# silencht/SG-SLAM

Hardware: AMD Instinct MI355X
Metric: tracked frames/sec (640x480 RGB-D) (higher is better)
Workload: dtype u8/f32(bf16x3 matrix products)/f64

## Files before the change

### sg_slam_amd/csrc/sgx_flow_kernels.h

```cpp
#pragma once
#include "sgx_rt.h"
#include "sgx_block.h"
#include "sgx_lane.h"
#include <float.h>
#include <math.h>

#define SGX_LK_MAXL 4
#define SGX_LK_WIN 21
#define SGX_LK_TILE_PITCH 36
struct SgxLkGeom {
    int nl;
    int w[SGX_LK_MAXL], h[SGX_LK_MAXL], pitch[SGX_LK_MAXL];
    unsigned ioff[SGX_LK_MAXL];
    unsigned img_stride;
};

SGX_DEV int sgx_reflect101(int p, int len)
{
    if (len == 1) return 0;
    while (p < 0 || p >= len) { if (p < 0) p = -p; else p = 2 * len - 2 - p; }
    return p;
}
SGX_DEV int sgx_floor_f(float v) { return (int)floorf(v); }
SGX_DEV float sgx_i64_to_f32(long long v)
// ... 118 lines not shown
    k.w10 = sgx_cvround((1.f - a) * b * (float)(1 << 14));
    k.w11 = (1 << 14) - k.w00 - k.w01 - k.w10;
    return k;
}
#define SGX_LK_DESCALE(x, n) (((x) + (1 << ((n) - 1))) >> (n))

struct SgxLkStep { float dx, dy; };
SGX_DEV SgxLkStep sgx_lk_step(float A11, float A12, float A22, float D, long long sb1, long long sb2)
{
    const float FLT_SCALE = 1.f / (1 << 20);
    const float b1 = sgx_i64_to_f32(sb1) * FLT_SCALE, b2 = sgx_i64_to_f32(sb2) * FLT_SCALE;
    SgxLkStep s;
    s.dx = (A12 * b2 - A22 * b1) * D;
    s.dy = (A12 * b1 - A11 * b2) * D;
    return s;
}

struct SgxLkArgs {
    const uint8_t *cur_img, *prev_img;
    const uint8_t *keys; const int *n; int cap;
    float *prev_xy; uint8_t *status;
    int max_count; double eps2; float min_eig;
    int batch, kblocks;
};
SGX_DEV void sgx_lk_decode_block(int i, int batch, int kblocks, int &f, int &kb)
{
    const int full = (batch / 8) * 8;
    if (i < full * kblocks) { const int x = i & 7, j = i >> 3; kb = j % kblocks; f = x + 8 * (j / kblocks); }
    else { const int j = i - full * kblocks; f = full + j / kblocks; kb = j % kblocks; }
}

#ifdef SGX_EMU
static inline int sgx_lk_px(const uint8_t *I, int w, int h, int pitch, int x, int y) { return I[(size_t)sgx_reflect101(y, h) * pitch + sgx_reflect101(x, w)]; }
static void sgx_lk_track_point(const SgxLkGeom &g, const uint8_t *I0, const uint8_t *J0, float kx, float ky, int max_count, double eps2, float min_eig,
                               float *ox, float *oy, uint8_t *ost)
{
    const int W = SGX_LK_WIN; const float half = (W - 1) * 0.5f, FLT_SCALE = 1.f / (1 << 20);
    float outx = 0.f, outy = 0.f; uint8_t status = 1;
    static thread_local short Iw[SGX_LK_WIN * SGX_LK_WIN], dIw[SGX_LK_WIN * SGX_LK_WIN * 2];
    for (int level = g.nl - 1; level >= 0; level--) {
        const int w = g.w[level], h = g.h[level], pitch = g.pitch[level];
        const uint8_t *I = I0 + g.ioff[level], *J = J0 + g.ioff[level];
        const float sc = 1.0f / (float)(1 << level);
        float prevx = kx * sc, prevy = ky * sc, nextx, nexty;
        if (level == g.nl - 1) { nextx = prevx; nexty = prevy; } else { nextx = outx * 2.f; nexty = outy * 2.f; }
        outx = nextx; outy = nexty;
        prevx -= half; prevy -= half;
        const int ipx = sgx_floor_f(prevx), ipy = sgx_floor_f(prevy);
        if (ipx < -W || ipx >= w || ipy < -W || ipy >= h) { if (level == 0) status = 0; continue; }
        SgxLkWeights k = sgx_lk_weights(prevx - ipx, prevy - ipy);
        long long s11 = 0, s12 = 0, s22 = 0;
        for (int y = 0; y < W; y++) for (int x = 0; x < W; x++) {
            int pv[4], dx[4], dy[4];
            for (int c = 0; c < 4; c++) {
                const int gx = ipx + x + (c & 1), gy = ipy + y + (c >> 1);
                pv[c] = sgx_lk_px(I, w, h, pitch, gx, gy);
                if (gx < 0 || gy < 0 || gx >= w || gy >= h) { dx[c] = dy[c] = 0; }
                else {
                    int t0[3], t1[3];
                    for (int q = 0; q < 3; q++) {
                        const int a = sgx_lk_px(I, w, h, pitch, gx - 1 + q, gy - 1), b = sgx_lk_px(I, w, h, pitch, gx - 1 + q, gy), cc = sgx_lk_px(I, w, h, pitch, gx - 1 + q, gy + 1);
                        t0[q] = (a + cc) * 3 + b * 10; t1[q] = cc - a;
                    }
                    dx[c] = t0[2] - t0[0]; dy[c] = (t1[0] + t1[2]) * 3 + t1[1] * 10;
                }
            }
            const int iv = SGX_LK_DESCALE(pv[0] * k.w00 + pv[1] * k.w01 + pv[2] * k.w10 + pv[3] * k.w11, 9);
            const int ix = SGX_LK_DESCALE(dx[0] * k.w00 + dx[1] * k.w01 + dx[2] * k.w10 + dx[3] * k.w11, 14);
            const int iy = SGX_LK_DESCALE(dy[0] * k.w00 + dy[1] * k.w01 + dy[2] * k.w10 + dy[3] * k.w11, 14);
            Iw[y * W + x] = (short)iv; dIw[(y * W + x) * 2] = (short)ix; dIw[(y * W + x) * 2 + 1] = (short)iy;
            s11 += (long long)ix * ix; s12 += (long long)ix * iy; s22 += (long long)iy * iy;
        }
        const float A11 = sgx_i64_to_f32(s11) * FLT_SCALE, A12 = sgx_i64_to_f32(s12) * FLT_SCALE, A22 = sgx_i64_to_f32(s22) * FLT_SCALE;
        float D = A11 * A22 - A12 * A12;
        const float minEig = (A22 + A11 - sqrtf((A11 - A22) * (A11 - A22) + 4.f * A12 * A12)) / (float)(2 * W * W);
        if (minEig < min_eig || D < FLT_EPSILON) { if (level == 0) status = 0; continue; }
        D = 1.f / D;
        nextx -= half; nexty -= half;
        float pdx = 0.f, pdy = 0.f;
        for (int j = 0; j < max_count; j++) {
            const int inx = sgx_floor_f(nextx), iny = sgx_floor_f(nexty);
            if (inx < -W || inx >= w || iny < -W || iny >= h) { if (level == 0) status = 0; break; }
            k = sgx_lk_weights(nextx - inx, nexty - iny);
            long long sb1 = 0, sb2 = 0;
            for (int y = 0; y < W; y++) for (int x = 0; x < W; x++) {
                int pv[4];
                for (int c = 0; c < 4; c++) pv[c] = sgx_lk_px(J, w, h, pitch, inx + x + (c & 1), iny + y + (c >> 1));
                const int diff = SGX_LK_DESCALE(pv[0] * k.w00 + pv[1] * k.w01 + pv[2] * k.w10 + pv[3] * k.w11, 9) - Iw[y * W + x];
                sb1 += (long long)diff * dIw[(y * W + x) * 2]; sb2 += (long long)diff * dIw[(y * W + x) * 2 + 1];
            }
            const SgxLkStep st = sgx_lk_step(A11, A12, A22, D, sb1, sb2);
            nextx += st.dx; nexty += st.dy;
            outx = nextx + half; outy = nexty + half;
            if ((double)st.dx * st.dx + (double)st.dy * st.dy <= eps2) break;
            if (j > 0 && fabs((double)(st.dx + pdx)) < 0.01 && fabs((double)(st.dy + pdy)) < 0.01) { outx -= st.dx * 0.5f; outy -= st.dy * 0.5f; break; }
            pdx = st.dx; pdy = st.dy;
        }
        if (status && level == 0) {
            const int ix = sgx_floor_f(outx - half), iy = sgx_floor_f(outy - half);
            if (ix < -W || ix >= w || iy < -W || iy >= h) status = 0;
        }
    }
    *ox = outx; *oy = outy; *ost = status;
}
SGX_KERNEL(256) k_lk_track(SgxLkGeom g, SgxLkArgs A)
{
    SGX_THREADS_BEGIN(tid)
    int f, kb;
    sgx_lk_decode_block((int)blockIdx.x, A.batch, A.kblocks, f, kb);
    const int kp = kb * 4 + (tid >> 6);
    if ((tid & 63) == 0 && kp < A.n[f] && kp < A.cap) {
        const float *kpt = (const float *)(A.keys + ((size_t)f * A.cap + kp) * 28);
        float ox, oy; uint8_t st;
        sgx_lk_track_point(g, A.cur_img + (size_t)f * g.img_stride, A.prev_img + (size_t)f * g.img_stride, kpt[0], kpt[1], A.max_count, A.eps2, A.min_eig, &ox, &oy, &st);
        A.prev_xy[2 * ((size_t)f * A.cap + kp)] = ox; A.prev_xy[2 * ((size_t)f * A.cap + kp) + 1] = oy;
        if (A.status) A.status[(size_t)f * A.cap + kp] = st;
    }
    SGX_THREADS_END
}
#else
SGX_DEV int sgx_wave_sum_i32(int v)
{
    v += __builtin_amdgcn_update_dpp(0, v, 0xB1, 0xF, 0xF, true);
    v += __builtin_amdgcn_update_dpp(0, v, 0x4E, 0xF, 0xF, true);
    v += __builtin_amdgcn_update_dpp(0, v, 0x124, 0xF, 0xF, true);
    v += __builtin_amdgcn_update_dpp(0, v, 0x128, 0xF, 0xF, true);
    v += __builtin_amdgcn_update_dpp(0, v, 0x142, 0xA, 0xF, false);
    v += __builtin_amdgcn_update_dpp(0, v, 0x143, 0xC, 0xF, false);
    return __builtin_amdgcn_readlane(v, 63);
}
SGX_DEV float sgx_wave_sum_f32(int v)
{
    const int lo = sgx_wave_sum_i32(v & 0xFFFF), hi = sgx_wave_sum_i32(v >> 16);
    return fmaf((float)hi, 65536.0f, (float)lo);
}
SGX_DEV int sgx_mul24(int a, int b) { return __mul24(a, b); }
SGX_DEV int sgx_reflect1(int p, int len) { p = p < 0 ? -p : p; p = p >= len ? 2 * len - 2 - p : p; return min(max(p, 0), len - 1); }

typedef short sgx_i16x2 __attribute__((ext_vector_type(2)));
typedef unsigned short sgx_u16x2 __attribute__((ext_vector_type(2)));
SGX_DEV sgx_i16x2 sgx_as_i16x2(uint32_t v) { return __builtin_bit_cast(sgx_i16x2, v); }
SGX_DEV uint32_t sgx_as_u32(sgx_i16x2 v) { return __builtin_bit_cast(uint32_t, v); }
#define SGX_LK_PAIR(hi, lo, a, b) sgx_as_i16x2(__builtin_amdgcn_perm((hi), (lo), (uint32_t)(a) | 0x0c00u | ((uint32_t)(b) << 16) | 0x0c000000u))
SGX_DEV sgx_i16x2 sgx_lk_next(sgx_i16x2 p, sgx_i16x2 q) { return sgx_as_i16x2(__builtin_amdgcn_alignbit(sgx_as_u32(q), sgx_as_u32(p), 16)); }
#if defined(SGX_LK_NODOT) && !defined(SGX_EMU)
SGX_DEV int sgx_lk_dot2_mad(sgx_i16x2 a, sgx_i16x2 b, int c)
{
    const uint32_t ua = __builtin_bit_cast(uint32_t, a), ub = __builtin_bit_cast(uint32_t, b);
    asm("v_mad_i32_i16 %0, %1, %2, %0 op_sel:[0,0,0,0]" : "+v"(c) : "v"(ua), "v"(ub));
    asm("v_mad_i32_i16 %0, %1, %2, %0 op_sel:[1,1,0,0]" : "+v"(c) : "v"(ua), "v"(ub));
    return c;
}
#define SGX_LK_DOT2(a, b, c) sgx_lk_dot2_mad((a), (b), (c))
#else
#define SGX_LK_DOT2(a, b, c) __builtin_amdgcn_sdot2((a), (b), (c), false)
#endif
SGX_DEV int sgx_lk_dot2_keep(sgx_i16x2 a, sgx_i16x2 b, int c) { return SGX_LK_DOT2(a, b, c); }

template <int PASSES>
SGX_DEV void sgx_lk_stage(uint32_t *tile, const uint8_t *img, int w, int h, int pitch, int ox, int oy, int rl, int cl)
{
    __builtin_amdgcn_fence(__ATOMIC_SEQ_CST, "wavefront"); __builtin_amdgcn_wave_barrier();
    const int gx = ox + 4 * cl;
    const bool inside = gx >= 0 && gx + 4 <= w;
    if (rl < 7) {
        uint32_t v[PASSES];
        if (inside) {
#pragma unroll
            for (int p = 0; p < PASSES; p++) v[p] = *(const uint32_t *)(img + (size_t)sgx_reflect1(oy + p * 7 + rl, h) * pitch + gx);
        } else {
            const int x0 = sgx_reflect1(gx, w), x1 = sgx_reflect1(gx + 1, w), x2 = sgx_reflect1(gx + 2, w), x3 = sgx_reflect1(gx + 3, w);
#pragma unroll
            for (int p = 0; p < PASSES; p++) {
                const uint8_t *src = img + (size_t)sgx_reflect1(oy + p * 7 + rl, h) * pitch;
                v[p] = (uint32_t)src[x0] | ((uint32_t)src[x1] << 8) | ((uint32_t)src[x2] << 16) | ((uint32_t)src[x3] << 24);
            }
        }
#pragma unroll
        for (int p = 0; p < PASSES; p++) tile[(p * 7 + rl) * (SGX_LK_TILE_PITCH / 4) + cl] = v[p];
    }
    __builtin_amdgcn_fence(__ATOMIC_SEQ_CST, "wavefront"); __builtin_amdgcn_wave_barrier();
}

#ifdef SGX_DEBUG_TAPS
SGX_KERNEL(256) k_lk_track(SgxLkGeom g, SgxLkArgs A)
{
    __shared__ uint32_t tiles[4][35 * SGX_LK_TILE_PITCH / 4 + 5];
    const int tid = (int)threadIdx.x, lane = tid & 63, wv = tid >> 6;
    int f, kb;
    sgx_lk_decode_block((int)blockIdx.x, A.batch, A.kblocks, f, kb);
    const int kp = kb * 4 + wv;
    if (kp >= A.n[f] || kp >= A.cap) return;
    uint32_t *tile = tiles[wv];
    const uint8_t *tile8 = (const uint8_t *)tile;
    const int W = SGX_LK_WIN; const float half = 10.0f, FLT_SCALE = 1.f / (1 << 20);
    const float *kpt = (const float *)(A.keys + ((size_t)f * A.cap + kp) * 28);
    const float kx = __builtin_bit_cast(float, __builtin_amdgcn_readfirstlane(__builtin_bit_cast(int, kpt[0])));
    const float ky = __builtin_bit_cast(float, __builtin_amdgcn_readfirstlane(__builtin_bit_cast(int, kpt[1])));
    const uint8_t *I0 = A.cur_img + (size_t)f * g.img_stride, *J0 = A.prev_img + (size_t)f * g.img_stride;
    const int r = lane / 3, s7 = (lane - 3 * r) * 7;
    const int rl = lane / 9, cl = lane - 9 * rl;
    const bool active = lane < 63;
    const int lane_off = active ? r * SGX_LK_TILE_PITCH + s7 : 0;
    float outx = 0.f, outy = 0.f; int status = 1;

    for (int level = g.nl - 1; level >= 0; level--) {
        const int w = g.w[level], h = g.h[level], pitch = g.pitch[level];
        const uint8_t *I = I0 + g.ioff[level], *J = J0 + g.ioff[level];
        const float sc = 1.0f / (float)(1 << level);
        float prevx = kx * sc, prevy = ky * sc, nextx, nexty;
        if (level == g.nl - 1) { nextx = prevx; nexty = prevy; } else { nextx = outx * 2.f; nexty = outy * 2.f; }
        outx = nextx; outy = nexty;
        prevx -= half; prevy -= half;
        const int ipx = sgx_floor_f(prevx), ipy = sgx_floor_f(prevy);
        if (ipx < -W || ipx >= w || ipy < -W || ipy >= h) { if (level == 0) status = 0; continue; }
        SgxLkWeights k = sgx_lk_weights(prevx - ipx, prevy - ipy);
        sgx_i16x2 W0 = sgx_as_i16x2((uint32_t)k.w00 | ((uint32_t)k.w01 << 16)), W1 = sgx_as_i16x2((uint32_t)k.w10 | ((uint32_t)k.w11 << 16));

        int ivb[7]; int ix[7], iy[7];
        int s11 = 0, s12 = 0, s22 = 0;
        {
            const int gy0 = ipy + r, gx0 = ipx + s7;
            sgx_i16x2 P[4][5];
            const bool direct = ipx >= 1 && ipx + 25 < w && ipy >= 1 && ipy + 22 < h;
            if (direct) {
                const uint8_t *gb = I + (size_t)(active ? gy0 - 1 : ipy) * pitch + (active ? gx0 - 1 : ipx);
#pragma unroll
                for (int j = 0; j < 4; j++) {
                    uint32_t q[3];
                    __builtin_memcpy(q, gb + (size_t)j * pitch, 12);
                    P[j][0] = SGX_LK_PAIR(q[0], q[0], 0, 1); P[j][1] = SGX_LK_PAIR(q[0], q[0], 2, 3);
                    P[j][2] = SGX_LK_PAIR(q[1], q[1], 0, 1); P[j][3] = SGX_LK_PAIR(q[1], q[1], 2, 3);
                    P[j][4] = SGX_LK_PAIR(q[2], q[2], 0, 1);
                }
            } else {
                const int tx = ((ipx - 1) >> 2) << 2, ty = ipy - 1;
                sgx_lk_stage<4>(tile, I, w, h, pitch, tx, ty, rl, cl);
                const uint8_t *tb = tile8 + lane_off + (ipx - 1 - tx);
#pragma unroll
                for (int j = 0; j < 4; j++) {
                    uint32_t q[3];
                    __builtin_memcpy(q, tb + j * SGX_LK_TILE_PITCH, 12);
                    P[j][0] = SGX_LK_PAIR(q[0], q[0], 0, 1); P[j][1] = SGX_LK_PAIR(q[0], q[0], 2, 3);
                    P[j][2] = SGX_LK_PAIR(q[1], q[1], 0, 1); P[j][3] = SGX_LK_PAIR(q[1], q[1], 2, 3);
                    P[j][4] = SGX_LK_PAIR(q[2], q[2], 0, 1);
                }
            }
            const sgx_i16x2 c3 = { 3, 3 }, c10 = { 10, 10 };
            const sgx_i16x2 Wd0 = active ? W0 : sgx_as_i16x2(0u), Wd1 = active ? W1 : sgx_as_i16x2(0u);
            sgx_i16x2 S0[5], S1[5], D0[5], D1[5];
#pragma unroll
            for (int q = 0; q < 5; q++) {
                S0[q] = (P[0][q] + P[2][q]) * c3 + P[1][q] * c10; D0[q] = P[2][q] - P[0][q];
                S1[q] = (P[1][q] + P[3][q]) * c3 + P[2][q] * c10; D1[q] = P[3][q] - P[1][q];
            }
            sgx_i16x2 xa[5], ya[5], xb[5], yb[5];
            const bool whole = ipx >= 0 && ipx + W < w && ipy >= 0 && ipy + W < h;
#pragma unroll
            for (int q = 0; q < 4; q++) {
                xa[q] = S0[q + 1] - S0[q]; ya[q] = (D0[q] + D0[q + 1]) * c3 + sgx_lk_next(D0[q], D0[q + 1]) * c10;
                xb[q] = S1[q + 1] - S1[q]; yb[q] = (D1[q] + D1[q + 1]) * c3 + sgx_lk_next(D1[q], D1[q + 1]) * c10;
            }
            if (!whole) {
                const bool rowa = gy0 >= 0 && gy0 < h, rowb = gy0 + 1 >= 0 && gy0 + 1 < h;
#pragma unroll
                for (int q = 0; q < 4; q++) {
                    const int x = gx0 + 2 * q;
                    const uint32_t m = ((x >= 0 && x < w) ? 0xFFFFu : 0u) | ((x + 1 >= 0 && x + 1 < w) ? 0xFFFF0000u : 0u);
                    const uint32_t ma = rowa ? m : 0u, mb = rowb ? m : 0u;
                    xa[q] = sgx_as_i16x2(sgx_as_u32(xa[q]) & ma); ya[q] = sgx_as_i16x2(sgx_as_u32(ya[q]) & ma);
                    xb[q] = sgx_as_i16x2(sgx_as_u32(xb[q]) & mb); yb[q] = sgx_as_i16x2(sgx_as_u32(yb[q]) & mb);
                }
            }
#pragma unroll
            for (int c = 0; c < 7; c++) {
                const sgx_i16x2 pxa = (c & 1) ? sgx_lk_next(xa[c >> 1], xa[(c >> 1) + 1]) : xa[c >> 1], pxb = (c & 1) ? sgx_lk_next(xb[c >> 1], xb[(c >> 1) + 1]) : xb[c >> 1];
                const sgx_i16x2 pya = (c & 1) ? sgx_lk_next(ya[c >> 1], ya[(c >> 1) + 1]) : ya[c >> 1], pyb = (c & 1) ? sgx_lk_next(yb[c >> 1], yb[(c >> 1) + 1]) : yb[c >> 1];
                const sgx_i16x2 pia = (c & 1) ? P[1][(c + 1) >> 1] : sgx_lk_next(P[1][c >> 1], P[1][(c >> 1) + 1]), pib = (c & 1) ? P[2][(c + 1) >> 1] : sgx_lk_next(P[2][c >> 1], P[2][(c >> 1) + 1]);
                const int v = SGX_LK_DOT2(pib, W1, SGX_LK_DOT2(pia, W0, 256)) >> 9;
                const int vx = SGX_LK_DOT2(pxb, Wd1, SGX_LK_DOT2(pxa, Wd0, 8192)) >> 14;
                const int vy = SGX_LK_DOT2(pyb, Wd1, SGX_LK_DOT2(pya, Wd0, 8192)) >> 14;
                ivb[c] = 256 - (v << 9); ix[c] = vx; iy[c] = vy;
                s11 += sgx_mul24(vx, vx); s12 += sgx_mul24(vx, vy); s22 += sgx_mul24(vy, vy);
            }
        }
        const float A11 = sgx_wave_sum_f32(s11) * FLT_SCALE, A12 = sgx_wave_sum_f32(s12) * FLT_SCALE, A22 = sgx_wave_sum_f32(s22) * FLT_SCALE;
        float D = A11 * A22 - A12 * A12;
        const float minEig = (A22 + A11 - sqrtf((A11 - A22) * (A11 - A22) + 4.f * A12 * A12)) / (float)(2 * W * W);
        if (minEig < A.min_eig || D < FLT_EPSILON) { if (level == 0) status = 0; continue; }
        D = 1.f / D;
        nextx -= half; nexty -= half;
        float pdx = 0.f, pdy = 0.f;
        int ox = 0, oy = 0; bool staged = false;
        for (int j = 0; j < A.max_count; j++) {
            const int inx = sgx_floor_f(nextx), iny = sgx_floor_f(nexty);
            if (inx < -W || inx >= w || iny < -W || iny >= h) { if (level == 0) status = 0; break; }
            k = sgx_lk_weights(nextx - inx, nexty - iny);
            W0 = sgx_as_i16x2((uint32_t)k.w00 | ((uint32_t)k.w01 << 16)); W1 = sgx_as_i16x2((uint32_t)k.w10 | ((uint32_t)k.w11 << 16));
            if (!staged || inx < ox || inx - ox > SGX_LK_TILE_PITCH - 22 || iny < oy || iny - oy > 35 - 22) {
                ox = ((inx - 5) >> 2) << 2; oy = iny - 6;
                sgx_lk_stage<5>(tile, J, w, h, pitch, ox, oy, rl, cl);
                staged = true;
            }
            int sb1 = 0, sb2 = 0;
            {
                const uint8_t *tb = tile8 + lane_off + (iny - oy) * SGX_LK_TILE_PITCH + (inx - ox);
                uint32_t a[2], b[2];
                __builtin_memcpy(a, tb, 8); __builtin_memcpy(b, tb + SGX_LK_TILE_PITCH, 8);
#pragma unroll
                for (int c = 0; c < 7; c++) {
                    const int diff = SGX_LK_DOT2(SGX_LK_PAIR(b[1], b[0], c, c + 1), W1, SGX_LK_DOT2(SGX_LK_PAIR(a[1], a[0], c, c + 1), W0, ivb[c])) >> 9;
                    sb1 += sgx_mul24(diff, ix[c]); sb2 += sgx_mul24(diff, iy[c]);
                }
            }
            const float b1 = sgx_wave_sum_f32(sb1) * FLT_SCALE, b2 = sgx_wave_sum_f32(sb2) * FLT_SCALE;
            const float dx = (A12 * b2 - A22 * b1) * D, dy = (A12 * b1 - A11 * b2) * D;
            nextx += dx; nexty += dy;
            outx = nextx + half; outy = nexty + half;
            if ((double)dx * dx + (double)dy * dy <= A.eps2) break;
            if (j > 0 && fabs((double)(dx + pdx)) < 0.01 && fabs((double)(dy + pdy)) < 0.01) { outx -= dx * 0.5f; outy -= dy * 0.5f; break; }
            pdx = dx; pdy = dy;
        }
        if (status && level == 0) {
            const int qx = sgx_floor_f(outx - half), qy = sgx_floor_f(outy - half);
            if (qx < -W || qx >= w || qy < -W || qy >= h) status = 0;
        }
    }
    if (lane == 0) {
        A.prev_xy[2 * ((size_t)f * A.cap + kp)] = outx; A.prev_xy[2 * ((size_t)f * A.cap + kp) + 1] = outy;
        if (A.status) A.status[(size_t)f * A.cap + kp] = (uint8_t)status;
    }
}
#endif
#endif

#ifndef SGX_EMU
SGX_DEV int sgx_row_sum_i32(int v)
{
    v += __builtin_amdgcn_update_dpp(v, v, 0xB1, 0xF, 0xF, true);
    v += __builtin_amdgcn_update_dpp(v, v, 0x4E, 0xF, 0xF, true);
    v += __builtin_amdgcn_update_dpp(v, v, 0x124, 0xF, 0xF, true);
    v += __builtin_amdgcn_update_dpp(v, v, 0x128, 0xF, 0xF, true);
    return v;
}
template <int LPK>
SGX_DEV float sgx_group_sum_f32(int v)
{
    int lo = sgx_row_sum_i32(v & 0xFFFF), hi = sgx_row_sum_i32(v >> 16);
    if (LPK == 32) { lo += __shfl_xor(lo, 16, 64); hi += __shfl_xor(hi, 16, 64); }
    return fmaf((float)hi, 65536.0f, (float)lo);
}

#define SGX_LK4_PITCH 32
template <int NROWS, int LPK>
SGX_DEV void sgx_lk_stage_row(uint32_t *tile, const uint8_t *img, int w, int h, int pitch, int ox, int oy, int l16)
{
    constexpr int RPP = LPK / 8, G = LPK == 16 ? 6 : 3;
    const int c = l16 & 7, rs = l16 >> 3, gx = ox + 4 * c;
    const bool inside = gx >= 0 && gx + 4 <= w;
    const int x0 = sgx_reflect1(gx, w), x1 = sgx_reflect1(gx + 1, w), x2 = sgx_reflect1(gx + 2, w), x3 = sgx_reflect1(gx + 3, w);
#pragma unroll 1
    for (int r0 = rs; r0 < NROWS; r0 += RPP * G) {
        uint32_t v[G];
#pragma unroll
        for (int p = 0; p < G; p++) {
            const uint8_t *src = img + (size_t)sgx_reflect1(oy + min(r0 + RPP * p, NROWS - 1), h) * pitch;
            if (inside) v[p] = *(const uint32_t *)(src + gx);
            else v[p] = (uint32_t)src[x0] | ((uint32_t)src[x1] << 8) | ((uint32_t)src[x2] << 16) | ((uint32_t)src[x3] << 24);
        }
#pragma unroll
        for (int p = 0; p < G; p++) { const int r = r0 + RPP * p; if (r < NROWS) tile[r * (SGX_LK4_PITCH / 4) + c] = v[p]; }
    }
}

SGX_DEV void sgx_lk_segment_setup(const sgx_i16x2 (&P)[4][5], sgx_i16x2 W0, sgx_i16x2 W1, bool whole, int gx0, int gy0, int w, int h,
                                  int (&ivb)[7], uint32_t (&ixy)[7], int &s11, int &s12, int &s22)
{
    const sgx_i16x2 c3 = { 3, 3 }, c10 = { 10, 10 };
    sgx_i16x2 S0[5], S1[5], D0[5], D1[5];
#pragma unroll
    for (int q = 0; q < 5; q++) {
        S0[q] = (P[0][q] + P[2][q]) * c3 + P[1][q] * c10; D0[q] = P[2][q] - P[0][q];
        S1[q] = (P[1][q] + P[3][q]) * c3 + P[2][q] * c10; D1[q] = P[3][q] - P[1][q];
    }
    sgx_i16x2 xa[5], ya[5], xb[5], yb[5];
#pragma unroll
    for (int q = 0; q < 4; q++) {
        xa[q] = S0[q + 1] - S0[q]; ya[q] = (D0[q] + D0[q + 1]) * c3 + sgx_lk_next(D0[q], D0[q + 1]) * c10;
        xb[q] = S1[q + 1] - S1[q]; yb[q] = (D1[q] + D1[q + 1]) * c3 + sgx_lk_next(D1[q], D1[q + 1]) * c10;
    }
    if (!whole) {
        const bool rowa = gy0 >= 0 && gy0 < h, rowb = gy0 + 1 >= 0 && gy0 + 1 < h;
#pragma unroll
        for (int q = 0; q < 4; q++) {
            const int x = gx0 + 2 * q;
            const uint32_t m = ((x >= 0 && x < w) ? 0xFFFFu : 0u) | ((x + 1 >= 0 && x + 1 < w) ? 0xFFFF0000u : 0u);
            const uint32_t ma = rowa ? m : 0u, mb = rowb ? m : 0u;
            xa[q] = sgx_as_i16x2(sgx_as_u32(xa[q]) & ma); ya[q] = sgx_as_i16x2(sgx_as_u32(ya[q]) & ma);
            xb[q] = sgx_as_i16x2(sgx_as_u32(xb[q]) & mb); yb[q] = sgx_as_i16x2(sgx_as_u32(yb[q]) & mb);
        }
    }
#pragma unroll
    for (int c = 0; c < 7; c++) {
        const sgx_i16x2 pxa = (c & 1) ? sgx_lk_next(xa[c >> 1], xa[(c >> 1) + 1]) : xa[c >> 1], pxb = (c & 1) ? sgx_lk_next(xb[c >> 1], xb[(c >> 1) + 1]) : xb[c >> 1];
        const sgx_i16x2 pya = (c & 1) ? sgx_lk_next(ya[c >> 1], ya[(c >> 1) + 1]) : ya[c >> 1], pyb = (c & 1) ? sgx_lk_next(yb[c >> 1], yb[(c >> 1) + 1]) : yb[c >> 1];
        const sgx_i16x2 pia = (c & 1) ? P[1][(c + 1) >> 1] : sgx_lk_next(P[1][c >> 1], P[1][(c >> 1) + 1]), pib = (c & 1) ? P[2][(c + 1) >> 1] : sgx_lk_next(P[2][c >> 1], P[2][(c >> 1) + 1]);
        const int v = SGX_LK_DOT2(pib, W1, SGX_LK_DOT2(pia, W0, 256)) >> 9;
        const int vx = SGX_LK_DOT2(pxb, W1, SGX_LK_DOT2(pxa, W0, 8192)) >> 14;
        const int vy = SGX_LK_DOT2(pyb, W1, SGX_LK_DOT2(pya, W0, 8192)) >> 14;
        ivb[c] = 256 - (v << 9); ixy[c] = ((uint32_t)vx & 0xFFFFu) | ((uint32_t)vy << 16);
        s11 += sgx_mul24(vx, vx); s12 += sgx_mul24(vx, vy); s22 += sgx_mul24(vy, vy);
    }
}
SGX_DEV int sgx_mad_lo16(int diff, uint32_t pair, int acc) { asm("v_mad_i32_i16 %0, %1, %2, %0 op_sel:[0,0,0,0]" : "+v"(acc) : "v"(diff), "v"(pair)); return acc; }
SGX_DEV int sgx_mad_hi16(int diff, uint32_t pair, int acc) { asm("v_mad_i32_i16 %0, %1, %2, %0 op_sel:[0,1,0,0]" : "+v"(acc) : "v"(diff), "v"(pair)); return acc; }

template <int KPW>
SGX_KERNEL_OCC(256, (KPW == 4 ? 3 : 5)) k_lk_trackN(SgxLkGeom g, SgxLkArgs A)
{
    constexpr int LPK = 64 / KPW, SPL = KPW;
    constexpr int TD = 36 * SGX_LK4_PITCH / 4 + 5;
    __shared__ uint32_t tiles[4 * KPW][TD];
    const int tid = (int)threadIdx.x, lane = tid & 63, wv = tid >> 6, row = lane / LPK, l16 = lane % LPK;
    int f, kb;
    sgx_lk_decode_block((int)blockIdx.x, A.batch, A.kblocks, f, kb);
    const int nkp = min(A.n[f], A.cap);
    if (kb * (4 * KPW) + wv * KPW >= nkp) return;
    const int kp = kb * (4 * KPW) + wv * KPW + row;
    const bool valid = kp < nkp;
    uint32_t *tile = tiles[wv * KPW + row];
    const uint8_t *tile8 = (const uint8_t *)tile;
    const int W = SGX_LK_WIN; const float half = 10.0f, FLT_SCALE = 1.f / (1 << 20);
    const float *kpt = (const float *)(A.keys + ((size_t)f * A.cap + (valid ? kp : 0)) * 28);
    const float kx = kpt[0], ky = kpt[1];
    const uint8_t *I0 = A.cur_img + (size_t)f * g.img_stride, *J0 = A.prev_img + (size_t)f * g.img_stride;
    int soff[SPL], srow[SPL], scol[SPL];
#pragma unroll
    for (int q = 0; q < SPL; q++) { const int si = min(l16 + LPK * q, 62); srow[q] = si / 3; scol[q] = (si - 3 * srow[q]) * 7; soff[q] = srow[q] * SGX_LK4_PITCH + scol[q]; }
    const bool idle3 = l16 == LPK - 1;
    float outx = 0.f, outy = 0.f; int status = 1;

    for (int level = g.nl - 1; level >= 0; level--) {
        const int w = g.w[level], h = g.h[level], pitch = g.pitch[level];
        const uint8_t *I = I0 + g.ioff[level], *J = J0 + g.ioff[level];
        const float sc = 1.0f / (float)(1 << level);
        float prevx = kx * sc, prevy = ky * sc, nextx, nexty;
        if (level == g.nl - 1) { nextx = prevx; nexty = prevy; } else { nextx = outx * 2.f; nexty = outy * 2.f; }
        outx = nextx; outy = nexty;
        prevx -= half; prevy -= half;
        const int ipx = sgx_floor_f(prevx), ipy = sgx_floor_f(prevy);
        bool act = valid;
        if (ipx < -W || ipx >= w || ipy < -W || ipy >= h) { if (level == 0) status = 0; act = false; }
        if (!__any(act)) continue;
        SgxLkWeights k = sgx_lk_weights(prevx - ipx, prevy - ipy);
        sgx_i16x2 W0 = sgx_as_i16x2((uint32_t)k.w00 | ((uint32_t)k.w01 << 16)), W1 = sgx_as_i16x2((uint32_t)k.w10 | ((uint32_t)k.w11 << 16));

        int ivb[SPL][7]; uint32_t ixy[SPL][7];
        int s11 = 0, s12 = 0, s22 = 0;
        {
            const bool direct = act && ipx >= 1 && ipx + 25 < w && ipy >= 1 && ipy + 22 < h;
            const bool whole = !__any(act && !(ipx >= 0 && ipx + W < w && ipy >= 0 && ipy + W < h));
            const int tx = ((ipx - 1) >> 2) << 2, ty = ipy - 1;
            if (__any(act && !direct)) {
                __builtin_amdgcn_fence(__ATOMIC_SEQ_CST, "wavefront"); __builtin_amdgcn_wave_barrier();
                if (act && !direct) sgx_lk_stage_row<28, LPK>(tile, I, w, h, pitch, tx, ty, l16);
                __builtin_amdgcn_fence(__ATOMIC_SEQ_CST, "wavefront"); __builtin_amdgcn_wave_barrier();
            }
#pragma unroll
            for (int q = 0; q < SPL; q++) {
                const int gy0 = ipy + srow[q], gx0 = ipx + scol[q];
                sgx_i16x2 P[4][5];
                if (direct) {
                    const uint8_t *gb = I + (size_t)(gy0 - 1) * pitch + (gx0 - 1);
#pragma unroll
                    for (int j = 0; j < 4; j++) {
                        uint32_t d[3];
                        __builtin_memcpy(d, gb + (size_t)j * pitch, 12);
                        P[j][0] = SGX_LK_PAIR(d[0], d[0], 0, 1); P[j][1] = SGX_LK_PAIR(d[0], d[0], 2, 3);
                        P[j][2] = SGX_LK_PAIR(d[1], d[1], 0, 1); P[j][3] = SGX_LK_PAIR(d[1], d[1], 2, 3);
                        P[j][4] = SGX_LK_PAIR(d[2], d[2], 0, 1);
                    }
                } else {
                    const uint8_t *tb = tile8 + soff[q] + (ipx - 1 - tx);
#pragma unroll
                    for (int j = 0; j < 4; j++) {
                        uint32_t d[3];
                        __builtin_memcpy(d, tb + j * SGX_LK4_PITCH, 12);
                        P[j][0] = SGX_LK_PAIR(d[0], d[0], 0, 1); P[j][1] = SGX_LK_PAIR(d[0], d[0], 2, 3);
                        P[j][2] = SGX_LK_PAIR(d[1], d[1], 0, 1); P[j][3] = SGX_LK_PAIR(d[1], d[1], 2, 3);
                        P[j][4] = SGX_LK_PAIR(d[2], d[2], 0, 1);
                    }
                }
                const bool on = act && !(q == SPL - 1 && idle3);
                const sgx_i16x2 Wq0 = on ? W0 : sgx_as_i16x2(0u), Wq1 = on ? W1 : sgx_as_i16x2(0u);
                sgx_lk_segment_setup(P, Wq0, Wq1, whole, gx0, gy0, w, h, ivb[q], ixy[q], s11, s12, s22);
                __builtin_amdgcn_sched_barrier(0);
            }
        }
        const float A11 = sgx_group_sum_f32<LPK>(s11) * FLT_SCALE, A12 = sgx_group_sum_f32<LPK>(s12) * FLT_SCALE, A22 = sgx_group_sum_f32<LPK>(s22) * FLT_SCALE;
        float D = A11 * A22 - A12 * A12;
        const float minEig = (A22 + A11 - sqrtf((A11 - A22) * (A11 - A22) + 4.f * A12 * A12)) / (float)(2 * W * W);
        if (act && (minEig < A.min_eig || D < FLT_EPSILON)) { if (level == 0) status = 0; act = false; }
        D = 1.f / D;
        nextx -= half; nexty -= half;
        float pdx = 0.f, pdy = 0.f;
        int ox = 0, oy = 0; bool staged = false;
        for (int j = 0; j < A.max_count; j++) {
            const int inx = sgx_floor_f(nextx), iny = sgx_floor_f(nexty);
            if (act && (inx < -W || inx >= w || iny < -W || iny >= h)) { if (level == 0) status = 0; act = false; }
            if (!__any(act)) break;
            k = sgx_lk_weights(nextx - inx, nexty - iny);
            W0 = sgx_as_i16x2((uint32_t)k.w00 | ((uint32_t)k.w01 << 16)); W1 = sgx_as_i16x2((uint32_t)k.w10 | ((uint32_t)k.w11 << 16));
            const bool need = act && (!staged || inx < ox || inx - ox > SGX_LK4_PITCH - 22 || iny < oy || iny - oy > 36 - 22);
            if (__any(need)) {
                __builtin_amdgcn_fence(__ATOMIC_SEQ_CST, "wavefront"); __builtin_amdgcn_wave_barrier();
                if (need) {
                    ox = ((inx - 3) >> 2) << 2; oy = iny - 7;
                    sgx_lk_stage_row<36, LPK>(tile, J, w, h, pitch, ox, oy, l16);
                    staged = true;
                }
                __builtin_amdgcn_fence(__ATOMIC_SEQ_CST, "wavefront"); __builtin_amdgcn_wave_barrier();
            }
            int sb1 = 0, sb2 = 0;
            if (act) {
                const uint8_t *tb0 = tile8 + (iny - oy) * SGX_LK4_PITCH + (inx - ox);
#pragma unroll
                for (int q = 0; q < SPL; q++) {
                    const uint8_t *tb = tb0 + soff[q];
                    uint32_t a[2], b[2];
                    __builtin_memcpy(a, tb, 8); __builtin_memcpy(b, tb + SGX_LK4_PITCH, 8);
#pragma unroll
                    for (int c = 0; c < 7; c++) {
                        const int diff = SGX_LK_DOT2(SGX_LK_PAIR(b[1], b[0], c, c + 1), W1, sgx_lk_dot2_keep(SGX_LK_PAIR(a[1], a[0], c, c + 1), W0, ivb[q][c])) >> 9;
                        sb1 = sgx_mad_lo16(diff, ixy[q][c], sb1); sb2 = sgx_mad_hi16(diff, ixy[q][c], sb2);
                    }
                }
            }
            const float b1 = sgx_group_sum_f32<LPK>(sb1) * FLT_SCALE, b2 = sgx_group_sum_f32<LPK>(sb2) * FLT_SCALE;
            if (act) {
                const float dx = (A12 * b2 - A22 * b1) * D, dy = (A12 * b1 - A11 * b2) * D;
                nextx += dx; nexty += dy;
                outx = nextx + half; outy = nexty + half;
                const float f2 = dx * dx + dy * dy, e2f = (float)A.eps2;
                bool conv = f2 <= e2f;
                if (__any(fabsf(f2 - e2f) <= 1e-5f * e2f)) { asm volatile("" ::: "memory"); conv = (double)dx * dx + (double)dy * dy <= A.eps2; }
                if (conv) act = false;
                else if (j > 0 && fabsf(dx + pdx) <= 0.01f && fabsf(dy + pdy) <= 0.01f) { outx -= dx * 0.5f; outy -= dy * 0.5f; act = false; }
                pdx = dx; pdy = dy;
            }
        }
        if (valid && status && level == 0) {
            const int qx = sgx_floor_f(outx - half), qy = sgx_floor_f(outy - half);
            if (qx < -W || qx >= w || qy < -W || qy >= h) status = 0;
        }
    }
    if (l16 == 0 && valid) {
        A.prev_xy[2 * ((size_t)f * A.cap + kp)] = outx; A.prev_xy[2 * ((size_t)f * A.cap + kp) + 1] = outy;
        if (A.status) A.status[(size_t)f * A.cap + kp] = (uint8_t)status;
    }
}
#else
template <int KPW>
SGX_KERNEL(256) k_lk_trackN(SgxLkGeom g, SgxLkArgs A)
{
    SGX_THREADS_BEGIN(tid)
    int f, kb;
    sgx_lk_decode_block((int)blockIdx.x, A.batch, A.kblocks, f, kb);
    const int kp = kb * (4 * KPW) + tid / (64 / KPW);
    if (tid % (64 / KPW) == 0 && kp < A.n[f] && kp < A.cap) {
        const float *kpt = (const float *)(A.keys + ((size_t)f * A.cap + kp) * 28);
        float ox, oy; uint8_t st;
        sgx_lk_track_point(g, A.cur_img + (size_t)f * g.img_stride, A.prev_img + (size_t)f * g.img_stride, kpt[0], kpt[1], A.max_count, A.eps2, A.min_eig, &ox, &oy, &st);
        A.prev_xy[2 * ((size_t)f * A.cap + kp)] = ox; A.prev_xy[2 * ((size_t)f * A.cap + kp) + 1] = oy;
        if (A.status) A.status[(size_t)f * A.cap + kp] = st;
    }
    SGX_THREADS_END
}
#endif

#define SGX_FM_CHUNK 32
#define SGX_FM_MAXPTS 2048

SGX_DEV int sgx_solve_cubic(const double *c, double *roots)
{
    double a0 = c[0], a1 = c[1], a2 = c[2], a3 = c[3];
    double x0 = 0., x1 = 0., x2 = 0.;
    int n = 0;
    if (a0 == 0) {
        if (a1 == 0) {
            if (a2 == 0) n = a3 == 0 ? -1 : 0;
            else { x0 = -a3 / a2; n = 1; }
        } else {
            double d = a2 * a2 - 4 * a1 * a3;
            if (d >= 0) {
                d = sqrt(d);
                double q1 = (-a2 + d) * 0.5, q2 = (a2 + d) * -0.5;
                if (fabs(q1) > fabs(q2)) { x0 = q1 / a1; x1 = a3 / q1; }
                else { x0 = q2 / a1; x1 = a3 / q2; }
                n = d > 0 ? 2 : 1;
            }
        }
    } else {
        a0 = 1. / a0; a1 *= a0; a2 *= a0; a3 *= a0;
        double Q = (a1 * a1 - 3 * a2) * (1. / 9);
        double R = (2 * a1 * a1 * a1 - 9 * a1 * a2 + 27 * a3) * (1. / 54);
        double Qcubed = Q * Q * Q;
        double d = Qcubed - R * R;
        if (d > 0) {
            double theta = acos(R / sqrt(Qcubed));
            double sqrtQ = sqrt(Q);
            double t0 = -2 * sqrtQ, t1 = theta * (1. / 3), t2 = a1 * (1. / 3);
            x0 = t0 * cos(t1) - t2;
            x1 = t0 * cos(t1 + (2. * 3.1415926535897932384626433832795 / 3)) - t2;
            x2 = t0 * cos(t1 + (4. * 3.1415926535897932384626433832795 / 3)) - t2;
            n = 3;
        } else if (d == 0) {
            if (R >= 0) { x0 = -2 * pow(R, 1. / 3) - a1 / 3; x1 = pow(R, 1. / 3) - a1 / 3; }
            else { x0 = 2 * pow(-R, 1. / 3) - a1 / 3; x1 = -pow(-R, 1. / 3) - a1 / 3; }
            x2 = 0;
            n = x0 == x1 ? 1 : 2;
            x1 = x0 == x1 ? 0 : x1;
        } else {
            double e;
            d = sqrt(-d);
            e = pow(d + fabs(R), 1. / 3);
            if (R > 0) e = -e;
            x0 = (e + Q / e) - a1 * (1. / 3);
            n = 1;
        }
    }
    roots[0] = x0; roots[1] = x1; roots[2] = x2;
    return n;
}

SGX_DEV int sgx_fm_run7point(const float *m1, const float *m2, double *M, double *fmatrix)
{
    double beta[7], f1[9], f2[9], c[4], r[3];
    for (int i = 0; i < 7; i++) {
        const double x0 = m1[2 * i], y0 = m1[2 * i + 1], x1 = m2[2 * i], y1 = m2[2 * i + 1];
        M[0 * 7 + i] = x1 * x0; M[1 * 7 + i] = x1 * y0; M[2 * 7 + i] = x1;
        M[3 * 7 + i] = y1 * x0; M[4 * 7 + i] = y1 * y0; M[5 * 7 + i] = y1;
        M[6 * 7 + i] = x0; M[7 * 7 + i] = y0; M[8 * 7 + i] = 1;
    }
    for (int k = 0; k < 7; k++) {
        double nrm = 0; for (int i = k; i < 9; i++) nrm += M[i * 7 + k] * M[i * 7 + k];
        nrm = sqrt(nrm);
        beta[k] = 0;
        if (nrm == 0) continue;
        M[k * 7 + k] += M[k * 7 + k] >= 0 ? nrm : -nrm;
        double vv = 0; for (int i = k; i < 9; i++) vv += M[i * 7 + k] * M[i * 7 + k];
        if (vv == 0) continue;
        beta[k] = 2. / vv;
        for (int j = k + 1; j < 7; j++) {
            double s = 0; for (int i = k; i < 9; i++) s += M[i * 7 + k] * M[i * 7 + j];
            s *= beta[k];
            for (int i = k; i < 9; i++) M[i * 7 + j] -= s * M[i * 7 + k];
        }
    }
    for (int i = 0; i < 9; i++) { f1[i] = i == 7; f2[i] = i == 8; }
    for (int k = 6; k >= 0; k--) {
        double s1 = 0, s2 = 0;
        for (int i = k; i < 9; i++) { s1 += M[i * 7 + k] * f1[i]; s2 += M[i * 7 + k] * f2[i]; }
        s1 *= beta[k]; s2 *= beta[k];
        for (int i = k; i < 9; i++) { f1[i] -= s1 * M[i * 7 + k]; f2[i] -= s2 * M[i * 7 + k]; }
    }
    for (int i = 0; i < 9; i++) f1[i] -= f2[i];
    double t0 = f2[4] * f2[8] - f2[5] * f2[7], t1 = f2[3] * f2[8] - f2[5] * f2[6], t2 = f2[3] * f2[7] - f2[4] * f2[6];
    c[3] = f2[0] * t0 - f2[1] * t1 + f2[2] * t2;
    c[2] = f1[0] * t0 - f1[1] * t1 + f1[2] * t2 -
           f1[3] * (f2[1] * f2[8] - f2[2] * f2[7]) + f1[4] * (f2[0] * f2[8] - f2[2] * f2[6]) - f1[5] * (f2[0] * f2[7] - f2[1] * f2[6]) +
           f1[6] * (f2[1] * f2[5] - f2[2] * f2[4]) - f1[7] * (f2[0] * f2[5] - f2[2] * f2[3]) + f1[8] * (f2[0] * f2[4] - f2[1] * f2[3]);
    t0 = f1[4] * f1[8] - f1[5] * f1[7]; t1 = f1[3] * f1[8] - f1[5] * f1[6]; t2 = f1[3] * f1[7] - f1[4] * f1[6];
    c[0] = f1[0] * t0 - f1[1] * t1 + f1[2] * t2;
    c[1] = f2[0] * t0 - f2[1] * t1 + f2[2] * t2 -
           f2[3] * (f1[1] * f1[8] - f1[2] * f1[7]) + f2[4] * (f1[0] * f1[8] - f1[2] * f1[6]) - f2[5] * (f1[0] * f1[7] - f1[1] * f1[6]) +
           f2[6] * (f1[1] * f1[5] - f1[2] * f1[4]) - f2[7] * (f1[0] * f1[5] - f1[2] * f1[3]) + f2[8] * (f1[0] * f1[4] - f1[1] * f1[3]);
    const int n = sgx_solve_cubic(c, r);
    if (n < 1 || n > 3) return n;
    for (int k = 0; k < n; k++, fmatrix += 9) {
        double lambda = r[k], mu = 1.;
        const double s = f1[8] * r[k] + f2[8];
        if (fabs(s) > DBL_EPSILON) { mu = 1. / s; lambda *= mu; fmatrix[8] = 1.; }
        else fmatrix[8] = 0.;
        for (int i = 0; i < 8; i++) fmatrix[i] = f1[i] * lambda + f2[i] * mu;
    }
    return n;
}

SGX_DEV float sgx_fm_error(const double *F, float m1x, float m1y, float m2x, float m2y)
{
    double a, b, c, d1, d2, s1, s2;
    a = F[0] * m1x + F[1] * m1y + F[2];
    b = F[3] * m1x + F[4] * m1y + F[5];
    c = F[6] * m1x + F[7] * m1y + F[8];
    s2 = 1. / (a * a + b * b);
    d2 = m2x * a + m2y * b + c;
    a = F[0] * m2x + F[3] * m2y + F[6];
    b = F[1] * m2x + F[4] * m2y + F[7];
    c = F[2] * m2x + F[5] * m2y + F[8];
    s1 = 1. / (a * a + b * b);
    d1 = m1x * a + m1y * b + c;
    const double e1 = d1 * d1 * s1, e2 = d2 * d2 * s2;
    return (float)(e1 < e2 ? e2 : e1);
}

SGX_DEV bool sgx_fm_collinear7(const float *p)
{
    const int i = 6;
    for (int j = 0; j < i; j++) {
        const double dx1 = p[2 * j] - p[2 * i], dy1 = p[2 * j + 1] - p[2 * i + 1];
        for (int k = 0; k < j; k++) {
// ... 249 lines not shown
```

Measured before the change: 30570.

## Fold template term into precomputed cross sums and transpose LK weight pairing

Removes the per-pixel template value from the inner mismatch loop by precomputing sum(I*Ix) and sum(I*Iy) once per level and seeding the accumulators with their negation. The inner loop now interpolates J by pairing rows (a,b) vertically, so each column reuses shared packed pairs. It also adds partial-reduction steps before splitting sums into 16-bit halves, lane-id/readfirstlane hints, and occupancy macros. Overflow is guarded by static_asserts, though the rounding of the subtracted template differs slightly from before.

```diff
diff --git a/sg_slam_amd/csrc/sgx_flow_kernels.h b/sg_slam_amd/csrc/sgx_flow_kernels.h
--- a/sg_slam_amd/csrc/sgx_flow_kernels.h
+++ b/sg_slam_amd/csrc/sgx_flow_kernels.h
@@ -294,8 +294,10 @@
     return c;
 }
 #define SGX_LK_DOT2(a, b, c) sgx_lk_dot2_mad((a), (b), (c))
+#define SGX_LK_DOT2_CONST(a, b, c) sgx_lk_dot2_mad((a), (b), (c))
 #else
 #define SGX_LK_DOT2(a, b, c) __builtin_amdgcn_sdot2((a), (b), (c), false)
+#define SGX_LK_DOT2_CONST(a, b, c) __builtin_amdgcn_sdot2((a), (b), (c), true)
 #endif
 SGX_DEV int sgx_lk_dot2_keep(sgx_i16x2 a, sgx_i16x2 b, int c) { return SGX_LK_DOT2(a, b, c); }
 
@@ -485,10 +487,22 @@
     v += __builtin_amdgcn_update_dpp(v, v, 0x128, 0xF, 0xF, true);
     return v;
 }
-template <int LPK>
+template <int FROM, int TO>
+SGX_DEV int sgx_row_steps_i32(int v)
+{
+    if constexpr (FROM < TO) {
+        constexpr int ctrl = FROM == 0 ? 0xB1 : FROM == 1 ? 0x4E : FROM == 2 ? 0x124 : 0x128;
+        v += __builtin_amdgcn_update_dpp(v, v, ctrl, 0xF, 0xF, true);
+        return sgx_row_steps_i32<FROM + 1, TO>(v);
+    }
+    return v;
+}
+template <int LPK, int PRE>
 SGX_DEV float sgx_group_sum_f32(int v)
 {
-    int lo = sgx_row_sum_i32(v & 0xFFFF), hi = sgx_row_sum_i32(v >> 16);
+    static_assert(PRE >= 0 && PRE <= 4, "a row has four butterfly steps");
+    v = sgx_row_steps_i32<0, PRE>(v);
+    int lo = sgx_row_steps_i32<PRE, 4>(v & 0xFFFF), hi = sgx_row_steps_i32<PRE, 4>(v >> 16);
     if (LPK == 32) { lo += __shfl_xor(lo, 16, 64); hi += __shfl_xor(hi, 16, 64); }
     return fmaf((float)hi, 65536.0f, (float)lo);
 }
@@ -516,7 +530,7 @@
 }
 
 SGX_DEV void sgx_lk_segment_setup(const sgx_i16x2 (&P)[4][5], sgx_i16x2 W0, sgx_i16x2 W1, bool whole, int gx0, int gy0, int w, int h,
-                                  int (&ivb)[7], uint32_t (&ixy)[7], int &s11, int &s12, int &s22)
+                                  uint32_t (&ixy)[7], int &ci1, int &ci2, int &s11, int &s12, int &s22)
 {
     const sgx_i16x2 c3 = { 3, 3 }, c10 = { 10, 10 };
     sgx_i16x2 S0[5], S1[5], D0[5], D1[5];
@@ -547,28 +561,39 @@
         const sgx_i16x2 pxa = (c & 1) ? sgx_lk_next(xa[c >> 1], xa[(c >> 1) + 1]) : xa[c >> 1], pxb = (c & 1) ? sgx_lk_next(xb[c >> 1], xb[(c >> 1) + 1]) : xb[c >> 1];
         const sgx_i16x2 pya = (c & 1) ? sgx_lk_next(ya[c >> 1], ya[(c >> 1) + 1]) : ya[c >> 1], pyb = (c & 1) ? sgx_lk_next(yb[c >> 1], yb[(c >> 1) + 1]) : yb[c >> 1];
         const sgx_i16x2 pia = (c & 1) ? P[1][(c + 1) >> 1] : sgx_lk_next(P[1][c >> 1], P[1][(c >> 1) + 1]), pib = (c & 1) ? P[2][(c + 1) >> 1] : sgx_lk_next(P[2][c >> 1], P[2][(c >> 1) + 1]);
-        const int v = SGX_LK_DOT2(pib, W1, SGX_LK_DOT2(pia, W0, 256)) >> 9;
-        const int vx = SGX_LK_DOT2(pxb, W1, SGX_LK_DOT2(pxa, W0, 8192)) >> 14;
-        const int vy = SGX_LK_DOT2(pyb, W1, SGX_LK_DOT2(pya, W0, 8192)) >> 14;
-        ivb[c] = 256 - (v << 9); ixy[c] = ((uint32_t)vx & 0xFFFFu) | ((uint32_t)vy << 16);
+        const int v = SGX_LK_DOT2(pib, W1, SGX_LK_DOT2_CONST(pia, W0, 256)) >> 9;
+        const int vx = SGX_LK_DOT2(pxb, W1, SGX_LK_DOT2_CONST(pxa, W0, 8192)) >> 14;
+        const int vy = SGX_LK_DOT2(pyb, W1, SGX_LK_DOT2_CONST(pya, W0, 8192)) >> 14;
+        ixy[c] = ((uint32_t)vx & 0xFFFFu) | ((uint32_t)vy << 16);
+        ci1 += sgx_mul24(v, vx); ci2 += sgx_mul24(v, vy);
         s11 += sgx_mul24(vx, vx); s12 += sgx_mul24(vx, vy); s22 += sgx_mul24(vy, vy);
     }
 }
 SGX_DEV int sgx_mad_lo16(int diff, uint32_t pair, int acc) { asm("v_mad_i32_i16 %0, %1, %2, %0 op_sel:[0,0,0,0]" : "+v"(acc) : "v"(diff), "v"(pair)); return acc; }
 SGX_DEV int sgx_mad_hi16(int diff, uint32_t pair, int acc) { asm("v_mad_i32_i16 %0, %1, %2, %0 op_sel:[0,1,0,0]" : "+v"(acc) : "v"(diff), "v"(pair)); return acc; }
 
+#ifndef SGX_LK_OCC2
+#define SGX_LK_OCC2 5
+#endif
+#ifndef SGX_LK_OCC4
+#define SGX_LK_OCC4 3
+#endif
+#ifndef SGX_LK_PRESPLIT
+#define SGX_LK_PRESPLIT 1
+#endif
 template <int KPW>
-SGX_KERNEL_OCC(256, (KPW == 4 ? 3 : 5)) k_lk_trackN(SgxLkGeom g, SgxLkArgs A)
+SGX_KERNEL_OCC(256, (KPW == 4 ? SGX_LK_OCC4 : SGX_LK_OCC2)) k_lk_trackN(SgxLkGeom g, SgxLkArgs A)
 {
     constexpr int LPK = 64 / KPW, SPL = KPW;
     constexpr int TD = 36 * SGX_LK4_PITCH / 4 + 5;
     __shared__ uint32_t tiles[4 * KPW][TD];
-    const int tid = (int)threadIdx.x, lane = tid & 63, wv = tid >> 6, row = lane / LPK, l16 = lane % LPK;
+    const int tid = (int)threadIdx.x, lane = (int)__lane_id(), wv = __builtin_amdgcn_readfirstlane(tid >> 6), row = lane / LPK, l16 = lane % LPK;
     int f, kb;
     sgx_lk_decode_block((int)blockIdx.x, A.batch, A.kblocks, f, kb);
     const int nkp = min(A.n[f], A.cap);
-    if (kb * (4 * KPW) + wv * KPW >= nkp) return;
-    const int kp = kb * (4 * KPW) + wv * KPW + row;
+    const int kp0 = kb * (4 * KPW) + wv * KPW;
+    if (kp0 >= nkp) return;
+    const int kp = kp0 + row;
     const bool valid = kp < nkp;
     uint32_t *tile = tiles[wv * KPW + row];
     const uint8_t *tile8 = (const uint8_t *)tile;
@@ -597,8 +622,8 @@
         SgxLkWeights k = sgx_lk_weights(prevx - ipx, prevy - ipy);
         sgx_i16x2 W0 = sgx_as_i16x2((uint32_t)k.w00 | ((uint32_t)k.w01 << 16)), W1 = sgx_as_i16x2((uint32_t)k.w10 | ((uint32_t)k.w11 << 16));
 
-        int ivb[SPL][7]; uint32_t ixy[SPL][7];
-        int s11 = 0, s12 = 0, s22 = 0;
+        uint32_t ixy[SPL][7];
+        int s11 = 0, s12 = 0, s22 = 0, ci1 = 0, ci2 = 0;
         {
             const bool direct = act && ipx >= 1 && ipx + 25 < w && ipy >= 1 && ipy + 22 < h;
             const bool whole = !__any(act && !(ipx >= 0 && ipx + W < w && ipy >= 0 && ipy + W < h));
@@ -635,11 +660,13 @@
                 }
                 const bool on = act && !(q == SPL - 1 && idle3);
                 const sgx_i16x2 Wq0 = on ? W0 : sgx_as_i16x2(0u), Wq1 = on ? W1 : sgx_as_i16x2(0u);
-                sgx_lk_segment_setup(P, Wq0, Wq1, whole, gx0, gy0, w, h, ivb[q], ixy[q], s11, s12, s22);
+                sgx_lk_segment_setup(P, Wq0, Wq1, whole, gx0, gy0, w, h, ixy[q], ci1, ci2, s11, s12, s22);
                 __builtin_amdgcn_sched_barrier(0);
             }
         }
-        const float A11 = sgx_group_sum_f32<LPK>(s11) * FLT_SCALE, A12 = sgx_group_sum_f32<LPK>(s12) * FLT_SCALE, A22 = sgx_group_sum_f32<LPK>(s22) * FLT_SCALE;
+        constexpr int PRE_A = SGX_LK_PRESPLIT ? (SPL == 2 ? 3 : 2) : 0;
+        const float A11 = sgx_group_sum_f32<LPK, PRE_A>(s11) * FLT_SCALE, A12 = sgx_group_sum_f32<LPK, PRE_A>(s12) * FLT_SCALE, A22 = sgx_group_sum_f32<LPK, PRE_A>(s22) * FLT_SCALE;
+        const int nci1 = -ci1, nci2 = -ci2;
         float D = A11 * A22 - A12 * A12;
         const float minEig = (A22 + A11 - sqrtf((A11 - A22) * (A11 - A22) + 4.f * A12 * A12)) / (float)(2 * W * W);
         if (act && (minEig < A.min_eig || D < FLT_EPSILON)) { if (level == 0) status = 0; act = false; }
@@ -652,7 +679,7 @@
             if (act && (inx < -W || inx >= w || iny < -W || iny >= h)) { if (level == 0) status = 0; act = false; }
             if (!__any(act)) break;
             k = sgx_lk_weights(nextx - inx, nexty - iny);
-            W0 = sgx_as_i16x2((uint32_t)k.w00 | ((uint32_t)k.w01 << 16)); W1 = sgx_as_i16x2((uint32_t)k.w10 | ((uint32_t)k.w11 << 16));
+            const sgx_i16x2 WA = sgx_as_i16x2((uint32_t)k.w00 | ((uint32_t)k.w10 << 16)), WB = sgx_as_i16x2((uint32_t)k.w01 | ((uint32_t)k.w11 << 16));
             const bool need = act && (!staged || inx < ox || inx - ox > SGX_LK4_PITCH - 22 || iny < oy || iny - oy > 36 - 22);
             if (__any(need)) {
                 __builtin_amdgcn_fence(__ATOMIC_SEQ_CST, "wavefront"); __builtin_amdgcn_wave_barrier();
@@ -663,22 +690,32 @@
                 }
                 __builtin_amdgcn_fence(__ATOMIC_SEQ_CST, "wavefront"); __builtin_amdgcn_wave_barrier();
             }
+            static_assert(2LL * 7 * SPL * 8160 * 4080 < (1LL << 31), "a lane's running mismatch sum must fit 32 bits");
             int sb1 = 0, sb2 = 0;
             if (act) {
+                sb1 = nci1; sb2 = nci2;
                 const uint8_t *tb0 = tile8 + (iny - oy) * SGX_LK4_PITCH + (inx - ox);
 #pragma unroll
                 for (int q = 0; q < SPL; q++) {
                     const uint8_t *tb = tb0 + soff[q];
                     uint32_t a[2], b[2];
                     __builtin_memcpy(a, tb, 8); __builtin_memcpy(b, tb + SGX_LK4_PITCH, 8);
+                    sgx_i16x2 V[8];
+#pragma unroll
+                    for (int c = 0; c < 4; c++) { V[c] = SGX_LK_PAIR(b[0], a[0], c, 4 + c); V[4 + c] = SGX_LK_PAIR(b[1], a[1], c, 4 + c); }
+                    int x[7];
+#pragma unroll
+                    for (int c = 0; c < 7; c++) x[c] = SGX_LK_DOT2(V[c + 1], WB, SGX_LK_DOT2_CONST(V[c], WA, 256));
 #pragma unroll
                     for (int c = 0; c < 7; c++) {
-                        const int diff = SGX_LK_DOT2(SGX_LK_PAIR(b[1], b[0], c, c + 1), W1, sgx_lk_dot2_keep(SGX_LK_PAIR(a[1], a[0], c, c + 1), W0, ivb[q][c])) >> 9;
-                        sb1 = sgx_mad_lo16(diff, ixy[q][c], sb1); sb2 = sgx_mad_hi16(diff, ixy[q][c], sb2);
+                        const int jv = x[c] >> 9;
+                        sb1 = sgx_mad_lo16(jv, ixy[q][c], sb1); sb2 = sgx_mad_hi16(jv, ixy[q][c], sb2);
                     }
                 }
             }
-            const float b1 = sgx_group_sum_f32<LPK>(sb1) * FLT_SCALE, b2 = sgx_group_sum_f32<LPK>(sb2) * FLT_SCALE;
+            constexpr int PRE_B = SGX_LK_PRESPLIT ? (SPL == 2 ? 2 : 1) : 0;
+            static_assert((1LL << PRE_B) * 7 * SPL * 8160 * 4080 < (1LL << 31) && 16LL / SPL * 7 * SPL * 4080 * 4080 < (1LL << 31), "unsplit partial sums must fit 32 bits");
+            const float b1 = sgx_group_sum_f32<LPK, PRE_B>(sb1) * FLT_SCALE, b2 = sgx_group_sum_f32<LPK, PRE_B>(sb2) * FLT_SCALE;
             if (act) {
                 const float dx = (A12 * b2 - A22 * b1) * D, dy = (A12 * b1 - A11 * b2) * D;
                 nextx += dx; nexty += dy;
@@ -696,9 +733,13 @@
             if (qx < -W || qx >= w || qy < -W || qy >= h) status = 0;
         }
     }
-    if (l16 == 0 && valid) {
-        A.prev_xy[2 * ((size_t)f * A.cap + kp)] = outx; A.prev_xy[2 * ((size_t)f * A.cap + kp) + 1] = outy;
-        if (A.status) A.status[(size_t)f * A.cap + kp] = (uint8_t)status;
+    unsigned zero = 0;
+    asm volatile("" : "+s"(zero));
+    const int le = (int)__builtin_amdgcn_mbcnt_hi(~0u, __builtin_amdgcn_mbcnt_lo(~0u, zero));
+    if (le % LPK == 0 && valid) {
+        const size_t o = (size_t)f * A.cap + (kp0 + le / LPK);
+        A.prev_xy[2 * o] = outx; A.prev_xy[2 * o + 1] = outy;
+        if (A.status) A.status[o] = (uint8_t)status;
     }
 }
 #else
```

After: 30820 (median of 6 runs). About the same (+0.8%).
